# rst-tu-dortmund/teb_local_planner

Measured on NVIDIA B200. Metric: TEB trajectories/sec (complete optimizeTEB: outer x inner LM iterations + cost), higher is better.
Workload: dtype f64

## Files before the change

teb_local_planner_b200/csrc/teb_cabi.cu:

```cuda
#include <cuda_runtime.h>

#include <cmath>
#include <cstdio>
#include <cstring>
#include <new>
#include <string>
#include <vector>

#include "teb_kernels.cuh"
#include "teb_linearize.cuh"
#include "teb_spec.cuh"
#include "teb_solve_warp.cuh"
#include "teb_solve_lat.cuh"
#include "teb_hsig.cuh"
#include "teb_comm.h"
#include <cstdlib>

using namespace tebgpu;

struct tebgpu_ctx {
  int device = 0;
  cudaStream_t stream = nullptr;
  cudaStream_t side = nullptr;
  cudaEvent_t ev_fork = nullptr, ev_join = nullptr, ev_s0 = nullptr;
// ... 4 lines not shown
  int32_t* defer = nullptr;
  double* d_fp = nullptr;
  double* d_pverts = nullptr;
  double* d_hsig = nullptr;
  TebGpuLimits lim{};
  TebParams params{};
  bool have_params = false;
  std::string err;
  int64_t launches = 0;
  int linearize_variant = 0;
  ncclComm_t comm = nullptr;
  int world = 1, rank = 0;
  int32_t* arrive = nullptr;
  int eval_mode = 2;
  double* d_gather = nullptr;
  struct GraphEntry { uint64_t key = 0; cudaGraphExec_t exec = nullptr; int64_t launches = 0; uint64_t stamp = 0; int spec_k = 0, spec_first = 0; };
  std::vector<GraphEntry> graphs;
  uint64_t graph_clock = 0;
  uint64_t params_version = 0;
  int graph_mode = 2;
  int warp_solver = 4;
  int ring = 0;
  int eval_v1 = 0;
  int ka_staged = 1;
  int last_spec_k = 0;
  int last_spec_first = 0;
  int spec_k = 0;
  int solver = 2;
  int MW = 1;
  int chunks = 1;
  double* Hb = nullptr;
  unsigned long long* assoc = nullptr;
  unsigned long long* assoc3 = nullptr;
  double* dyn_t = nullptr;
  int32_t* via_idx = nullptr;
  double* chi_parts = nullptr;
  double* dmax_parts = nullptr;
  double* rhs = nullptr;
  int32_t* dyn_idx = nullptr;
  int32_t* dyn_cnt = nullptr;
  SpecBufs spec{};
  int eval_minb = 3;
  BandState* state = nullptr;
  double* d_poses = nullptr; int32_t* d_n = nullptr; int32_t* d_scene = nullptr; TebObstacle* d_obst = nullptr;
  int32_t* d_ocount = nullptr; double* d_via = nullptr; int32_t* d_vcount = nullptr; double* d_vs = nullptr;
  double* d_vg = nullptr; int32_t* d_rot = nullptr; double* d_cost = nullptr; double* d_chi2 = nullptr;
  int32_t* d_status = nullptr; int32_t* d_iters = nullptr;
// ... 203 lines not shown
  CUDA_TRY(c, cudaMalloc(&c->d_pverts, (S * (size_t)(lim->max_obst_vertices > 0 ? lim->max_obst_vertices : 1)) * 2 * sizeof(double)));
  CUDA_TRY(c, cudaMalloc(&c->d_hsig, B * (M > 2 ? M : 2) * sizeof(double)));
  CUDA_TRY(c, cudaMalloc(&c->d_vcount, B * sizeof(int32_t)));
  CUDA_TRY(c, cudaMalloc(&c->d_vs, B * 4 * sizeof(double)));
  CUDA_TRY(c, cudaMalloc(&c->d_vg, B * 4 * sizeof(double)));
  CUDA_TRY(c, cudaMalloc(&c->d_rot, B * sizeof(int32_t)));
  CUDA_TRY(c, cudaMalloc(&c->d_cost, B * sizeof(double)));
  CUDA_TRY(c, cudaMalloc(&c->d_chi2, B * sizeof(double)));
  CUDA_TRY(c, cudaMalloc(&c->d_status, B * sizeof(int32_t)));
  CUDA_TRY(c, cudaMalloc(&c->d_iters, B * sizeof(int32_t)));
  CUDA_TRY(c, cudaMemsetAsync(c->dyn_t, 0, B * nc * sizeof(double), c->stream));
  CUDA_TRY(c, cudaMemsetAsync(c->via_idx, 0xff, B * V * sizeof(int32_t), c->stream));
  c->smem_a = ka_smem_bytes((int)M);
  c->smem_b = kb_smem_bytes((int)nc, (int)M);
  c->smem_g = M * sizeof(TebObstacle);
  if (c->smem_b > 232448 || c->smem_a > 232448) {
    c->err = "shared-memory footprint exceeds 227 KB for these limits (max_poses / max_obstacles too large)";
    return TEBGPU_ERR_CAPACITY;
  }
  if (ka2_smem_bytes<true>((int)M) > 232448) {
    c->err = "kernel A staging exceeds 227 KB for these limits (max_obstacles too large)";
    return TEBGPU_ERR_CAPACITY;
  }
#define KA2_ATTR(H, G, O)                                                                                                    \
  CUDA_TRY(c, cudaFuncSetAttribute(k_linearize2<H, G, O>, cudaFuncAttributeMaxDynamicSharedMemorySize, (int)ka2_smem_bytes<H>((int)M))); \
  CUDA_TRY(c, cudaFuncSetAttribute(k_linearize2<H, G, O>, cudaFuncAttributePreferredSharedMemoryCarveout, cudaSharedmemCarveoutMaxShared));
  KA2_ATTR(false, false, true) KA2_ATTR(false, true, true) KA2_ATTR(true, false, true) KA2_ATTR(true, true, true)
  KA2_ATTR(false, false, false) KA2_ATTR(false, true, false) KA2_ATTR(true, false, false) KA2_ATTR(true, true, false)
#undef KA2_ATTR
  c->ka_staged = 1;
  if (const char* e = std::getenv("TEBGPU_KA_STAGED")) c->ka_staged = std::atoi(e) != 0;
  CUDA_TRY(c, cudaFuncSetAttribute(k_linearize<false, false>, cudaFuncAttributeMaxDynamicSharedMemorySize, (int)c->smem_a));
  CUDA_TRY(c, cudaFuncSetAttribute(k_linearize<false, true>, cudaFuncAttributeMaxDynamicSharedMemorySize, (int)c->smem_a));
  CUDA_TRY(c, cudaFuncSetAttribute(k_linearize<true, false>, cudaFuncAttributeMaxDynamicSharedMemorySize, (int)c->smem_a));
  CUDA_TRY(c, cudaFuncSetAttribute(k_linearize<true, true>, cudaFuncAttributeMaxDynamicSharedMemorySize, (int)c->smem_a));
  CUDA_TRY(c, cudaFuncSetAttribute(k_lm_step_t<0, KB_THREADS, false>, cudaFuncAttributeMaxDynamicSharedMemorySize, (int)c->smem_b));
  CUDA_TRY(c, cudaFuncSetAttribute(k_lm_step_t<0, KB_THREADS, true>, cudaFuncAttributeMaxDynamicSharedMemorySize, (int)c->smem_b));
  if ((int)nc <= BCR_MAX_POSES && kb_bcr_smem_bytes((int)nc, (int)M) <= 232448) {
    CUDA_TRY(c, cudaFuncSetAttribute(k_lm_step_t<1, KB_BCR_THREADS, false>, cudaFuncAttributeMaxDynamicSharedMemorySize,
                                     (int)kb_bcr_smem_bytes((int)nc, (int)M)));
    CUDA_TRY(c, cudaFuncSetAttribute(k_lm_step_t<1, KB_BCR_THREADS, true>, cudaFuncAttributeMaxDynamicSharedMemorySize,
                                     (int)kb_bcr_smem_bytes((int)nc, (int)M)));
  }
  CUDA_TRY(c, cudaFuncSetAttribute(k_build_graph<false>, cudaFuncAttributeMaxDynamicSharedMemorySize, (int)c->smem_g));
  CUDA_TRY(c, cudaFuncSetAttribute(k_build_graph<true>, cudaFuncAttributeMaxDynamicSharedMemorySize, (int)c->smem_g));
  CUDA_TRY(c, cudaFuncSetAttribute(k_linearize<false, false>, cudaFuncAttributePreferredSharedMemoryCarveout, cudaSharedmemCarveoutMaxShared));
  CUDA_TRY(c, cudaFuncSetAttribute(k_linearize<false, true>, cudaFuncAttributePreferredSharedMemoryCarveout, cudaSharedmemCarveoutMaxShared));
  CUDA_TRY(c, cudaFuncSetAttribute(k_linearize<true, false>, cudaFuncAttributePreferredSharedMemoryCarveout, cudaSharedmemCarveoutMaxShared));
  CUDA_TRY(c, cudaFuncSetAttribute(k_linearize<true, true>, cudaFuncAttributePreferredSharedMemoryCarveout, cudaSharedmemCarveoutMaxShared));
  CUDA_TRY(c, cudaFuncSetAttribute(k_solve_tpb<10>, cudaFuncAttributePreferredSharedMemoryCarveout, cudaSharedmemCarveoutMaxShared));
  CUDA_TRY(c, cudaFuncSetAttribute(k_solve_tpb<20>, cudaFuncAttributePreferredSharedMemoryCarveout, cudaSharedmemCarveoutMaxShared));
  CUDA_TRY(c, cudaFuncSetAttribute(k_solve_tpb<30>, cudaFuncAttributePreferredSharedMemoryCarveout, cudaSharedmemCarveoutMaxShared));
  CUDA_TRY(c, cudaFuncSetAttribute(k_solve_tpb<20>, cudaFuncAttributeMaxDynamicSharedMemorySize, tpb_ring_bytes(20)));
  CUDA_TRY(c, cudaFuncSetAttribute(k_solve_tpb<30>, cudaFuncAttributeMaxDynamicSharedMemorySize, tpb_ring_bytes(30)));
// ... 49 lines not shown
  for (int k = 0; k < 4; ++k) fp[FP_LINE + k] = p->footprint_line[k];
  fp[FP_COUNT] = (double)p->footprint_vertex_count;
  for (int k = 0; k < 2 * TEB_MAX_FOOTPRINT_VERTICES; ++k) fp[FP_VERTS + k] = p->footprint_vertices[k];
  CUDA_TRY(ctx, cudaSetDevice(ctx->device));
  CUDA_TRY(ctx, cudaStreamSynchronize(ctx->stream));
  CUDA_TRY(ctx, cudaMemcpy(ctx->d_fp, fp, sizeof(fp), cudaMemcpyHostToDevice));
  ctx->params = *p;
  ctx->have_params = true;
  ++ctx->params_version;
  return TEBGPU_OK;
}

static void launch_linearize(tebgpu_ctx* ctx, const DevBatch& db, const KParams& kp, int B, int M_cap, cudaStream_t st) {
  const bool holo = kp.holo_vel || kp.holo_acc;
  const bool geom = kp.generic != 0;
  if (ctx->linearize_variant == 1) {
    const dim3 grid(db.chunks, B);
    const size_t sm = ka_smem_bytes(M_cap);
    if (holo && geom) k_linearize<true, true><<<grid, KA_THREADS, sm, st>>>(db, kp);
    else if (holo) k_linearize<true, false><<<grid, KA_THREADS, sm, st>>>(db, kp);
    else if (geom) k_linearize<false, true><<<grid, KA_THREADS, sm, st>>>(db, kp);
    else k_linearize<false, false><<<grid, KA_THREADS, sm, st>>>(db, kp);
  } else {
    const dim3 g2((db.chunks + KA2_W - 1) / KA2_W, B);
    const size_t sm = holo ? ka2_smem_bytes<true>(M_cap) : ka2_smem_bytes<false>(M_cap);
#define KA2_LAUNCH(H, G)                                                                      \
  do {                                                                                        \
    if (ctx->ka_staged) k_linearize2<H, G, false><<<g2, KA2_THREADS, sm, st>>>(db, kp);       \
    else k_linearize2<H, G, true><<<g2, KA2_THREADS, sm, st>>>(db, kp);                       \
  } while (0)
    if (holo && geom) KA2_LAUNCH(true, true);
    else if (holo) KA2_LAUNCH(true, false);
    else if (geom) KA2_LAUNCH(false, true);
    else KA2_LAUNCH(false, false);
#undef KA2_LAUNCH
  }
}
static void launch_build_graph(const DevBatch& db, const KParams& kp, int B, size_t smem, cudaStream_t st) {
  if (kp.generic) k_build_graph<true><<<B, 256, smem, st>>>(db, kp);
  else k_build_graph<false><<<B, 256, smem, st>>>(db, kp);
}
static void launch_vor(const DevBatch& db, const KParams& kp, int B, size_t smem, cudaStream_t st) {
  if (kp.generic) k_vor<true><<<B, 256, smem, st>>>(db, kp);
  else k_vor<false><<<B, 256, smem, st>>>(db, kp);
}
static size_t eval_bytes(const tebgpu_ctx* ctx, int n_cap, int M_cap, int K) {
  return ctx->eval_v1 ? eval_smem_bytes(n_cap, M_cap, K) : eval2_smem_bytes(n_cap, M_cap, K);
}
static void launch_trial_eval(tebgpu_ctx* ctx, const SpecBufs& spec, const DevBatch& db, const KParams& kp, int B, int K,
                              size_t smem, int it, int round, int g, int tag, cudaStream_t st) {
  const size_t smem3 = eval3_smem_bytes(db.n_cap, db.M_cap, K);
  if (!ctx->eval_v1 && smem3 <= 232448 && (ctx->eval_mode == 1 || (ctx->eval_mode == 2 && (long long)B * K <= 148 * 3))) {
    int warps = ev2_tiles(db.n_cap);
    warps = warps < 1 ? 1 : (warps > 16 ? 16 : warps);
    const dim3 grid(K, B);
    if (kp.generic) k_trial_eval3<true><<<grid, 32 * warps, smem3, st>>>(db, kp, spec, it, round, g, tag, ctx->arrive);
    else k_trial_eval3<false><<<grid, 32 * warps, smem3, st>>>(db, kp, spec, it, round, g, tag, ctx->arrive);
    return;
// ... 262 lines not shown
        else if (kp.generic) k_lm_step_t<0, KB_THREADS, true><<<B, KB_THREADS, smem_b, st>>>(db, kp, it);
        else k_lm_step_t<0, KB_THREADS, false><<<B, KB_THREADS, smem_b, st>>>(db, kp, it);
        ++launches; prof_end(ctx, st);
      }
    }
    weight_multiplier *= p.weight_adapt_factor;
  }
  prof_begin(ctx, st, 5); k_finalize<<<gb, tb, 0, st>>>(db, kp, *args); ++launches; prof_end(ctx, st);
  ctx->launches = launches;
  if (ctx->profiling && ctx->ev_used > 4096) { cudaStreamSynchronize(st); prof_collect(ctx); }
  CUDA_TRY(ctx, cudaGetLastError());
  return TEBGPU_OK;
}

static uint64_t graph_key(const tebgpu_ctx* ctx, const TebBatch* bt, const TebOptimizeArgs* a, cudaStream_t st) {
  uint64_t h = 1469598103934665603ull;
  auto mix = [&](const void* p, size_t nbytes) {
    const unsigned char* c = static_cast<const unsigned char*>(p);
    for (size_t k = 0; k < nbytes; ++k) { h ^= c[k]; h *= 1099511628211ull; }
  };
  mix(bt, sizeof(*bt));
  mix(a, sizeof(*a));
  mix(&ctx->params_version, sizeof(ctx->params_version));
  const int sw[11] = {ctx->solver, ctx->spec_k, ctx->linearize_variant, ctx->ka_staged, ctx->eval_v1, ctx->ring, ctx->overlap, ctx->eval_minb, ctx->warp_solver, ctx->eval_mode, ctx->split};
  mix(sw, sizeof(sw));
  mix(&st, sizeof(st));
  return h;
}

int32_t tebgpu_optimize_batch_device(tebgpu_ctx* ctx, const TebBatch* bt, const TebOptimizeArgs* args, void* cuda_stream) {
  int32_t rc = check_batch(ctx, bt);
  if (rc) return rc;
  if (!args || args->iterations_innerloop < 0 || args->iterations_outerloop < 0) { ctx->err = "bad optimize args"; return TEBGPU_ERR_INVALID_ARG; }
  CUDA_TRY(ctx, cudaSetDevice(ctx->device));
  cudaStream_t st = cuda_stream ? (cudaStream_t)cuda_stream : ctx->stream;
  const bool latency_regime = (long long)bt->B * 8 <= 148LL * 4 * 32;
  const bool use_graph = !ctx->profiling && (ctx->graph_mode == 1 || (ctx->graph_mode == 2 && latency_regime));
  if (!use_graph) return issue_optimize(ctx, bt, args, st);
  const uint64_t key = graph_key(ctx, bt, args, st);
  for (auto& e : ctx->graphs)
    if (e.key == key) {
      e.stamp = ++ctx->graph_clock;
      ctx->launches = e.launches;
      ctx->last_spec_k = e.spec_k; ctx->last_spec_first = e.spec_first;
      CUDA_TRY(ctx, cudaGraphLaunch(e.exec, st));
      return TEBGPU_OK;
    }
// ... 431 lines not shown
```

teb_local_planner_b200/csrc/teb_linearize.cuh:

```cuda
#pragma once

#include "teb_kernels.cuh"

namespace tebgpu {

constexpr int KA2_W = 4;
constexpr int KA2_THREADS = 32 * KA2_W;
constexpr int KA2_TP = 29;
constexpr int KA2_SLOTS = KA2_W * KA2_TP + 4;
constexpr int KA2_NT = 32;
constexpr int OUT_STRIDE = 50;

template <bool HOLO>
struct JL {
  static constexpr int V = 0;
  static constexpr int W = V + 7;
  static constexpr int K0 = W + 3;
  static constexpr int K1 = K0 + 6;
  static constexpr int SP = K1 + 6;
  static constexpr int ROT = SP + 4;
  static constexpr int VY = ROT + 2;
  static constexpr int A0 = VY + (HOLO ? 6 : 0);
  static constexpr int A1 = A0 + 11;
  static constexpr int A2 = A1 + 5;
  static constexpr int E = A2 + (HOLO ? 11 : 0);
  static constexpr int COUNT = E + (HOLO ? 10 : 8);
};
constexpr unsigned M_V = 0x7Fu, M_W = (1u << 2) | (1u << 3) | (1u << 6), M_K = 0x77u, M_SP = 0x33u,
                   M_ROT = (1u << 2) | (1u << 6), M_VY = 0x3Fu, M_A0 = 0x7FFu,
                   M_A1 = (1u << 2) | (1u << 3) | (1u << 6) | (1u << 7) | (1u << 10);
enum { E_V = 0, E_W = 1, E_K0 = 2, E_K1 = 3, E_SP = 4, E_ROT = 5, E_A0 = 6, E_A1 = 7, E_VY = 8, E_A2 = 9 };

__host__ __device__ constexpr int cidx(unsigned mask, int col) {
  int k = 0;
  for (int c = 0; c < col; ++c) k += (mask >> c) & 1u;
  return k;
}

struct JRec {
  double* rec;
  template <int BASE, unsigned MASK, int COL>
  __device__ __forceinline__ void set(double v) const {
    if constexpr ((MASK >> COL) & 1u) rec[(BASE + cidx(MASK, COL)) * KA2_NT] = v;
  }
  __device__ __forceinline__ void res(int base_e, int k, double v) const { rec[(base_e + k) * KA2_NT] = v; }
};

struct KA2Smem {
  static constexpr int POSES = KA2_SLOTS * 4;
  static constexpr int START = 24;
  template <bool HOLO>
  __host__ __device__ static constexpr int rec_doubles() {
    return JL<HOLO>::COUNT * 32 > OUT_STRIDE * 32 ? JL<HOLO>::COUNT * 32 : OUT_STRIDE * 32;
  }
  template <bool HOLO>
  __host__ __device__ static constexpr int warp_doubles() { return rec_doubles<HOLO>() + START; }
};
template <bool HOLO>
__host__ __device__ inline size_t ka2_smem_bytes(int M_cap) {
  const size_t d = KA2Smem::POSES + (size_t)KA2_W * KA2Smem::warp_doubles<HOLO>() + 2;
  return d * sizeof(double) + (size_t)(M_cap > 0 ? M_cap : 1) * sizeof(TebObstacle) + 64;
}

template <bool HOLO>
__device__ __forceinline__ double anchor_rows2(const KParams& kp, const DevBatch& db, int b, int a, int n,
                                               const double* pa , double ca, double sa, double cb,
                                               double sb, const SegDer& sd, const SegDer& sd2, const JRec J,
                                               double* sStart) {
  using L = JL<HOLO>;
  const double* pb = pa + 4;
  const double v1 = sd.v, w1 = sd.w, idt1 = sd.idt;
  const double dx = pb[0] - pa[0], dy = pb[1] - pa[1];
  const bool fa = (a == 0), fb = (a + 1 == n - 1);
  const double ma = fa ? 0.0 : 1.0, mb = fb ? 0.0 : 1.0;
  double csum = 0;
  if (HOLO && kp.has_vel && kp.holo_vel) {
    const HoloDer h = holo_derivs(pa[0], pa[1], pa[2], ca, sa, pb[0], pb[1], pb[2], pa[3]);
    double e[3], sl[3], c0, c1;
    holo_velocity_terms(kp, h.vx, h.vy, h.w, e, sl, c0, c1);
    const double kx = kp.sw_vel_x, ky = kp.sw_vel_y, kw = kp.sw_vel_th * sl[2];
    J.set<L::V, M_V, 0>(ma * kx * (sl[0] * h.dvx[0] - c0 * h.dvy[0]));
    J.set<L::V, M_V, 1>(ma * kx * (sl[0] * h.dvx[1] - c0 * h.dvy[1]));
    J.set<L::V, M_V, 2>(ma * kx * (sl[0] * h.dvx[2] - c0 * h.dvy[2]));
// ... 225 lines not shown
      if (vs[3] != 0) {
        const double acc = (v1 - vs[0]) * idt1;
        const double accr = (w1 - vs[2]) * idt1;
        double s0, s1;
        const double e0 = pen_interval(acc, kp.p.acc_lim_x, kp.p.penalty_epsilon, s0);
        const double e1 = pen_interval(accr, kp.p.acc_lim_theta, kp.p.penalty_epsilon, s1);
        const double k0 = kp.sw_acc_x * s0 * idt1, k1 = kp.sw_acc_th * s1 * idt1;
        double* S0 = sStart;
        double* S1 = sStart + 7;
        S0[0] = 0; S0[1] = 0; S0[2] = 0;
        S0[3] = k0 * (-v1 * idt1 - acc);
        S0[4] = k0 * sd.dv[3] * mb; S0[5] = k0 * sd.dv[4] * mb; S0[6] = k0 * sd.dv[5] * mb;
        S1[0] = S1[1] = S1[2] = S1[4] = S1[5] = 0;
        S1[3] = k1 * (-w1 * idt1 - accr);
        S1[6] = k1 * idt1 * mb;
        sStart[START_E] = kp.sw_acc_x * e0; sStart[START_E + 1] = kp.sw_acc_th * e1;
        csum += sStart[START_E] * sStart[START_E] + sStart[START_E + 1] * sStart[START_E + 1];
      }
    }
  }
  return csum;
}

template <int D, int BASE, unsigned MASK, int NC>
__device__ __forceinline__ void gram_row(const double* __restrict__ jr_base, double e, double (&acc)[4][11], double (&brow)[4]) {
  constexpr int LMAX = (4 * D + 3 < NC - 1) ? 4 * D + 3 : NC - 1;
  if constexpr (4 * D < NC) {
    double jr[NC];
#pragma unroll
    for (int col = 0; col < NC; ++col) jr[col] = (((MASK >> col) & 1u) && col <= LMAX) ? jr_base[(BASE + cidx(MASK, col)) * KA2_NT] : 0.0;
#pragma unroll
    for (int c = 0; c < 4; ++c) {
      const int l = 4 * D + c;
      if (l < NC && ((MASK >> l) & 1u)) {
        const double jl = jr[l];
        brow[c] -= jl * e;
#pragma unroll
        for (int o = 0; o <= 10; ++o) {
          const int col = l - o;
          if (col >= 0 && ((MASK >> col) & 1u)) acc[c][o] += jl * jr[col];
        }
      }
    }
  }
}

template <bool HOLO, int D>
__device__ __forceinline__ void gram_anchor(const KParams& kp, const double* __restrict__ jr_base, double (&acc)[4][11],
                                            double (&brow)[4]) {
  using L = JL<HOLO>;
  const double* E = jr_base + L::E * KA2_NT;
  if (D < 2) {
    if (kp.has_vel) {
      const double ev = E[E_V * KA2_NT], ew = E[E_W * KA2_NT];
      if (ev != 0) gram_row<D, L::V, M_V, 7>(jr_base, ev, acc, brow);
      if (ew != 0) gram_row<D, L::W, M_W, 7>(jr_base, ew, acc, brow);
      if (HOLO) {
        const double ey = E[E_VY * KA2_NT];
        if (ey != 0) gram_row<D, L::VY, M_VY, 6>(jr_base, ey, acc, brow);
      }
    }
    if (kp.has_kin) {
      const double e0 = E[E_K0 * KA2_NT], e1 = E[E_K1 * KA2_NT];
      if (e0 != 0) gram_row<D, L::K0, M_K, 7>(jr_base, e0, acc, brow);
      if (e1 != 0) gram_row<D, L::K1, M_K, 7>(jr_base, e1, acc, brow);
    }
    if (kp.has_sp) {
      const double e = E[E_SP * KA2_NT];
      if (e != 0) gram_row<D, L::SP, M_SP, 6>(jr_base, e, acc, brow);
    }
    if (kp.has_rot) {
      const double e = E[E_ROT * KA2_NT];
      if (e != 0) gram_row<D, L::ROT, M_ROT, 7>(jr_base, e, acc, brow);
    }
  }
  if (kp.has_acc) {
    const double e0 = E[E_A0 * KA2_NT], e1 = E[E_A1 * KA2_NT];
    if (e0 != 0) gram_row<D, L::A0, M_A0, 11>(jr_base, e0, acc, brow);
    if (e1 != 0) gram_row<D, L::A1, M_A1, 11>(jr_base, e1, acc, brow);
    if (HOLO) {
      const double e2 = E[E_A2 * KA2_NT];
      if (e2 != 0) gram_row<D, L::A2, M_A0, 11>(jr_base, e2, acc, brow);
    }
  }
}

template <bool HOLO, int D>
__device__ __forceinline__ void gram_start(const double* sStart, double (&acc)[4][11], double (&brow)[4]) {
#pragma unroll
  for (int k = 0; k < (HOLO ? 3 : 2); ++k) {
    const double e = sStart[START_E + k];
    if (e == 0) continue;
#pragma unroll
    for (int c = 0; c < 4; ++c) {
      const int l = 4 * D + c;
      if (l <= 6) {
        const double jl = sStart[7 * k + l];
        brow[c] -= jl * e;
#pragma unroll
        for (int o = 0; o <= 6; ++o)
          if (o <= l) acc[c][o] += jl * sStart[7 * k + l - o];
      }
    }
  }
}

template <bool GEOM>
__device__ __forceinline__ void unary_terms2(const KParams& kp, const DevBatch& db, int b, int sc, int i, int n, double px,
                                             double py, double cs, double sn, const TebObstacle* so, unsigned long long mask0,
                                             double U[6], double ub[3], double& chi_obst, double& chi_via) {
  if (i < 1 || i > n - 2) return;
  const double* pool = db.obst_vertices + (size_t)sc * db.PV_cap * 2;
  if (kp.has_obst) {
    const unsigned long long* assoc = db.assoc + ((size_t)b * db.n_cap + i) * db.MW;
    for (int w = 0; w < db.MW; ++w) {
      unsigned long long mask = (w == 0) ? mask0 : assoc[w];
      while (mask) {
        const int m = (w << 6) + __ffsll((long long)mask) - 1;
        mask &= mask - 1;
        const TebObstacle ob = so[m];
        double g[3], kappa, beta;
        const double d = robot_obstacle_distance<GEOM>(kp, pool, px, py, cs, sn, ob, ob.x, ob.y, 0.0, 0.0, g);
        double cterm = obstacle_terms(kp, d, kappa, beta);
        if (kp.p.legacy_obstacle_association &&
            ((db.assoc3[((size_t)b * db.n_cap + i) * db.MW + w] >> (m & 63)) & 1ull)) {
          cterm *= 3; kappa *= 3; beta *= 3;
        }
        chi_obst += cterm;
        if (kappa != 0 || beta != 0) {
          U[0] += kappa * g[0] * g[0]; U[1] += kappa * g[0] * g[1]; U[2] += kappa * g[1] * g[1];
          U[3] += kappa * g[0] * g[2]; U[4] += kappa * g[1] * g[2]; U[5] += kappa * g[2] * g[2];
          ub[0] -= beta * g[0]; ub[1] -= beta * g[1]; ub[2] -= beta * g[2];
        }
      }
    }
  }
  if (kp.has_dyn) {
    const double t = db.dyn_t[(size_t)b * db.n_cap + i];
    const int nd = db.dyn_cnt[sc];
    const int32_t* di = db.dyn_idx + (size_t)sc * db.M_cap;
    for (int q = 0; q < nd; ++q) {
      const TebObstacle ob = so[di[q]];
      double g[3], kappa, beta;
      const double d = robot_obstacle_distance<GEOM>(kp, pool, px, py, cs, sn, ob, ob.x + t * ob.vx, ob.y + t * ob.vy, t * ob.vx,
                                               t * ob.vy, g);
      chi_obst += dynamic_terms(kp, d, kappa, beta);
      if (kappa != 0 || beta != 0) {
        U[0] += kappa * g[0] * g[0]; U[1] += kappa * g[0] * g[1]; U[2] += kappa * g[1] * g[1];
        U[3] += kappa * g[0] * g[2]; U[4] += kappa * g[1] * g[2]; U[5] += kappa * g[2] * g[2];
        ub[0] -= beta * g[0]; ub[1] -= beta * g[1]; ub[2] -= beta * g[2];
      }
    }
  }
  if (kp.has_via && db.V_cap > 0) {
    const int32_t* vidx = db.via_idx + (size_t)b * db.V_cap;
    const double* via = db.via + (size_t)b * db.V_cap * 2;
    const double wv = kp.p.weight_viapoint;
    for (int v = 0; v < db.V_cap; ++v) {
      if (vidx[v] != i) continue;
      const double dx = px - via[2 * v], dy = py - via[2 * v + 1];
      const double e = sqrt(dx * dx + dy * dy);
      chi_via += wv * e * e;
      if (e > 0) {
        const double gx = dx / e, gy = dy / e;
        U[0] += wv * gx * gx; U[1] += wv * gx * gy; U[2] += wv * gy * gy;
        ub[0] -= wv * e * gx; ub[1] -= wv * e * gy;
      }
    }
  }
}

__device__ __forceinline__ double shfl_down1(double v) { return __shfl_down_sync(0xffffffffu, v, 1); }

template <bool HOLO, bool GEOM, bool OUT_DIRECT>
__global__ void __launch_bounds__(KA2_THREADS, 3) k_linearize2(const __grid_constant__ DevBatch db, const __grid_constant__ KParams kp) {
  extern __shared__ __align__(128) unsigned char smem_raw[];
  using L = JL<HOLO>;
  const int tid = threadIdx.x, lane = tid & 31, warp = tid >> 5;
  double* sP = reinterpret_cast<double*>(smem_raw);
  double* sW = sP + KA2Smem::POSES + (size_t)warp * KA2Smem::warp_doubles<HOLO>();
  double* sStart = sW + KA2Smem::rec_doubles<HOLO>();
  uint64_t* bar = reinterpret_cast<uint64_t*>(sP + KA2Smem::POSES + (size_t)KA2_W * KA2Smem::warp_doubles<HOLO>());
  TebObstacle* so = reinterpret_cast<TebObstacle*>((reinterpret_cast<uintptr_t>(bar) + 16 + 15) & ~static_cast<uintptr_t>(15));

  const int y = blockIdx.y;
  int b = y, skip = 0;
  if (db.a_list) { if (y < *db.a_cnt) b = db.a_list[y]; else skip = 1; }
  else if (db.skip_tag != 0 && deferred_since(db.defer[y], db.skip_tag)) skip = 1;
  if (skip) return;
  const int active = db.state[b].active;
  const int n = db.n[b];
  const int s = db.scene_id[b];
  const int P0 = blockIdx.x * (KA2_W * KA2_TP) - 2;
  const int lo = max(P0, 0), hi = min(P0 + KA2_SLOTS, db.n_cap);
  if (tid == 0) {
    mbar_init(bar, 1);
    mbar_fence_init();
  }
  if (!active || P0 + 2 >= n) return;
  if (tid == 0) {
    const uint32_t bytesP = (uint32_t)(hi - lo) * 32u;
    const uint32_t bytesO = (uint32_t)db.M_cap * (uint32_t)sizeof(TebObstacle);
    mbar_expect_tx(bar, bytesP + bytesO);
    tma_load_1d(sP + (size_t)(lo - P0) * 4, db.poses + ((size_t)b * db.n_cap + lo) * 4, bytesP, bar);
    if (bytesO) tma_load_1d(so, db.obstacles + (size_t)s * db.M_cap, bytesO, bar);
  }
  const int slot = warp * KA2_TP + lane;
  const int i = P0 + slot;
  const int q0 = P0 + 2 + warp * KA2_TP;
  const bool out = (lane >= 2 && lane <= 30 && i < n);
  unsigned long long mask0 = 0ull;
  if (out && kp.has_obst && i >= 1 && i <= n - 2) mask0 = db.assoc[((size_t)b * db.n_cap + i) * db.MW];
  {
    double* rec = sW + lane;
#pragma unroll
    for (int e = 0; e < L::COUNT; ++e) rec[e * 32] = 0.0;
    if (lane < KA2Smem::START) sStart[lane] = 0.0;
  }
  __syncthreads();
  mbar_wait(bar, 0);
  if (q0 >= n) return;

  double chi[4] = {0, 0, 0, 0};
  const bool have_pose = (i >= 0 && i < n);
  const double* pa = sP + 4 * slot;
  double cs = 1, sn = 0;
  SegDer sd;
  sd.v = 0; sd.w = 0; sd.idt = 0;
#pragma unroll
  for (int k = 0; k < 6; ++k) sd.dv[k] = 0;
  double U[6] = {0, 0, 0, 0, 0, 0}, ub[3] = {0, 0, 0};
  if (have_pose) {
    sincos(pa[2], &sn, &cs);
    if (i <= n - 2) sd = seg_derivs(kp, pa[0], pa[1], pa[2], cs, sn, pa[4], pa[5], pa[6], pa[3]);
    if (out) unary_terms2<GEOM>(kp, db, b, s, i, n, pa[0], pa[1], cs, sn, so, mask0, U, ub, chi[0], chi[1]);
  }
  SegDer sd2;
  const double cb = shfl_down1(cs), sb = shfl_down1(sn);
  sd2.v = shfl_down1(sd.v); sd2.w = shfl_down1(sd.w); sd2.idt = shfl_down1(sd.idt);
#pragma unroll
  for (int k = 0; k < 6; ++k) sd2.dv[k] = shfl_down1(sd.dv[k]);
  __syncwarp();
  if (have_pose && i <= n - 2 && lane < 31) {
    JRec J;
    J.rec = sW + lane;
    const double c3 = anchor_rows2<HOLO>(kp, db, b, i, n, pa, cs, sn, cb, sb, sd, sd2, J, sStart);
    if (lane >= 2) chi[3] += c3;
  }
  __syncwarp();
  double acc[4][11];
  double brow[4] = {0, 0, 0, 0};
#pragma unroll
  for (int c = 0; c < 4; ++c)
#pragma unroll
    for (int k = 0; k < 11; ++k) acc[c][k] = 0;
  double dm = 0;
  if (out) {
    const double* rec = sW + lane;
    if (i <= n - 2) gram_anchor<HOLO, 0>(kp, rec, acc, brow);
    if (i >= 1) gram_anchor<HOLO, 1>(kp, rec - 1, acc, brow);
    if (i >= 2) gram_anchor<HOLO, 2>(kp, rec - 2, acc, brow);
    if (kp.has_acc) {
      if (i == 0) gram_start<HOLO, 0>(sStart, acc, brow);
      if (i == 1) gram_start<HOLO, 1>(sStart, acc, brow);
    }
    acc[0][0] += U[0]; brow[0] += ub[0];
    acc[1][0] += U[2]; acc[1][1] += U[1]; brow[1] += ub[1];
    acc[2][0] += U[5]; acc[2][1] += U[4]; acc[2][2] += U[3]; brow[2] += ub[2];
    if (kp.has_time && i <= n - 2) {
      chi[2] += kp.p.weight_optimaltime * pa[3] * pa[3];
      acc[3][0] += kp.p.weight_optimaltime; brow[3] -= kp.p.weight_optimaltime * pa[3];
    }
    if (i == 0 || i >= n - 1) {
#pragma unroll
      for (int c = 0; c < 4; ++c) {
        if (c == 3 && i <= n - 2) continue;
#pragma unroll
        for (int k = 0; k < 11; ++k) acc[c][k] = 0;
        acc[c][0] = 1.0;
        brow[c] = 0;
      }
      dm = (i <= n - 2) ? fabs(acc[3][0]) : 0.0;
    } else {
      dm = fmax(fmax(fabs(acc[0][0]), fabs(acc[1][0])), fmax(fabs(acc[2][0]), fabs(acc[3][0])));
    }
  }
  if (OUT_DIRECT) {
    if (out) {
      double2* g2 = reinterpret_cast<double2*>(db.Hb + ((size_t)b * 4 * db.n_cap + 4 * (size_t)i) * HROW);
#pragma unroll
      for (int c = 0; c < 4; ++c) {
#pragma unroll
        for (int k = 0; k < 5; ++k) g2[6 * c + k] = make_double2(acc[c][2 * k], acc[c][2 * k + 1]);
        g2[6 * c + 5] = make_double2(acc[c][10], brow[c]);
      }
      double2* r2 = reinterpret_cast<double2*>(db.rhs + (size_t)b * 4 * db.n_cap + 4 * (size_t)i);
      r2[0] = make_double2(brow[0], brow[1]);
      r2[1] = make_double2(brow[2], brow[3]);
    }
  } else {
    __syncwarp();
    if (out) {
      double2* o2 = reinterpret_cast<double2*>(sW + (size_t)lane * OUT_STRIDE);
#pragma unroll
      for (int c = 0; c < 4; ++c) {
#pragma unroll
        for (int k = 0; k < 5; ++k) o2[6 * c + k] = make_double2(acc[c][2 * k], acc[c][2 * k + 1]);
        o2[6 * c + 5] = make_double2(acc[c][10], brow[c]);
      }
      double2* r2 = reinterpret_cast<double2*>(db.rhs + (size_t)b * 4 * db.n_cap + 4 * (size_t)i);
      r2[0] = make_double2(brow[0], brow[1]);
      r2[1] = make_double2(brow[2], brow[3]);
      fence_proxy_async();
      tma_store_1d(db.Hb + ((size_t)b * 4 * db.n_cap + 4 * (size_t)i) * HROW, o2, 4 * HROW * 8u);
      asm volatile("cp.async.bulk.commit_group;" ::: "memory");
    }
  }
  {
#pragma unroll
    for (int k = 0; k < 4; ++k) chi[k] = warp_sum(chi[k]);
    dm = warp_max(dm);
    if (lane == 0) {
      const int tile = blockIdx.x * KA2_W + warp;
      double* cp = db.chi_parts + ((size_t)b * db.chunks + tile) * 4;
      cp[0] = chi[0]; cp[1] = chi[1]; cp[2] = chi[2]; cp[3] = chi[3];
      db.dmax_parts[(size_t)b * db.chunks + tile] = dm;
    }
  }
  if (!OUT_DIRECT && out) asm volatile("cp.async.bulk.wait_group.read 0;" ::: "memory");
}

}
```

Before: 171,100.

## Split linearize tile work across warp pairs with role-specialized warps

Restructures the linearization kernel so each 29-pose tile is handled by a pair of warps instead of one. One warp computes the segment derivatives and anchor Jacobian rows, while the other computes the obstacle unary terms. Each warp then builds two of the four Gram rows and writes them with its own bulk store. Named barriers and a shared exchange buffer pass the unary block and the diagonal max between the two warps. The change also evaluates obstacles two at a time for more instruction-level parallelism, raises the min-CTA launch bounds, and drops the direct-output variant and its environment switch. It aims to cut per-thread register pressure and serial latency, at the cost of more shared memory, extra barriers and more CTAs.

```diff
diff --git a/teb_local_planner_b200/csrc/teb_cabi.cu b/teb_local_planner_b200/csrc/teb_cabi.cu
--- a/teb_local_planner_b200/csrc/teb_cabi.cu
+++ b/teb_local_planner_b200/csrc/teb_cabi.cu
@@ -50,7 +50,6 @@
   int warp_solver = 4;
   int ring = 0;
   int eval_v1 = 0;
-  int ka_staged = 1;
   int last_spec_k = 0;
   int last_spec_first = 0;
   int spec_k = 0;
@@ -300,14 +299,11 @@
     c->err = "kernel A staging exceeds 227 KB for these limits (max_obstacles too large)";
     return TEBGPU_ERR_CAPACITY;
   }
-#define KA2_ATTR(H, G, O)                                                                                                    \
-  CUDA_TRY(c, cudaFuncSetAttribute(k_linearize2<H, G, O>, cudaFuncAttributeMaxDynamicSharedMemorySize, (int)ka2_smem_bytes<H>((int)M))); \
-  CUDA_TRY(c, cudaFuncSetAttribute(k_linearize2<H, G, O>, cudaFuncAttributePreferredSharedMemoryCarveout, cudaSharedmemCarveoutMaxShared));
-  KA2_ATTR(false, false, true) KA2_ATTR(false, true, true) KA2_ATTR(true, false, true) KA2_ATTR(true, true, true)
-  KA2_ATTR(false, false, false) KA2_ATTR(false, true, false) KA2_ATTR(true, false, false) KA2_ATTR(true, true, false)
+#define KA2_ATTR(H, G)                                                                                                    \
+  CUDA_TRY(c, cudaFuncSetAttribute(k_linearize2<H, G>, cudaFuncAttributeMaxDynamicSharedMemorySize, (int)ka2_smem_bytes<H>((int)M))); \
+  CUDA_TRY(c, cudaFuncSetAttribute(k_linearize2<H, G>, cudaFuncAttributePreferredSharedMemoryCarveout, cudaSharedmemCarveoutMaxShared));
+  KA2_ATTR(false, false) KA2_ATTR(false, true) KA2_ATTR(true, false) KA2_ATTR(true, true)
 #undef KA2_ATTR
-  c->ka_staged = 1;
-  if (const char* e = std::getenv("TEBGPU_KA_STAGED")) c->ka_staged = std::atoi(e) != 0;
   CUDA_TRY(c, cudaFuncSetAttribute(k_linearize<false, false>, cudaFuncAttributeMaxDynamicSharedMemorySize, (int)c->smem_a));
   CUDA_TRY(c, cudaFuncSetAttribute(k_linearize<false, true>, cudaFuncAttributeMaxDynamicSharedMemorySize, (int)c->smem_a));
   CUDA_TRY(c, cudaFuncSetAttribute(k_linearize<true, false>, cudaFuncAttributeMaxDynamicSharedMemorySize, (int)c->smem_a));
@@ -403,18 +399,12 @@
     else if (geom) k_linearize<false, true><<<grid, KA_THREADS, sm, st>>>(db, kp);
     else k_linearize<false, false><<<grid, KA_THREADS, sm, st>>>(db, kp);
   } else {
-    const dim3 g2((db.chunks + KA2_W - 1) / KA2_W, B);
+    const dim3 g2((db.chunks + KA2_P - 1) / KA2_P, B);
     const size_t sm = holo ? ka2_smem_bytes<true>(M_cap) : ka2_smem_bytes<false>(M_cap);
-#define KA2_LAUNCH(H, G)                                                                      \
-  do {                                                                                        \
-    if (ctx->ka_staged) k_linearize2<H, G, false><<<g2, KA2_THREADS, sm, st>>>(db, kp);       \
-    else k_linearize2<H, G, true><<<g2, KA2_THREADS, sm, st>>>(db, kp);                       \
-  } while (0)
-    if (holo && geom) KA2_LAUNCH(true, true);
-    else if (holo) KA2_LAUNCH(true, false);
-    else if (geom) KA2_LAUNCH(false, true);
-    else KA2_LAUNCH(false, false);
-#undef KA2_LAUNCH
+    if (holo && geom) k_linearize2<true, true><<<g2, KA2_THREADS, sm, st>>>(db, kp);
+    else if (holo) k_linearize2<true, false><<<g2, KA2_THREADS, sm, st>>>(db, kp);
+    else if (geom) k_linearize2<false, true><<<g2, KA2_THREADS, sm, st>>>(db, kp);
+    else k_linearize2<false, false><<<g2, KA2_THREADS, sm, st>>>(db, kp);
   }
 }
 static void launch_build_graph(const DevBatch& db, const KParams& kp, int B, size_t smem, cudaStream_t st) {
@@ -723,7 +713,7 @@
   mix(bt, sizeof(*bt));
   mix(a, sizeof(*a));
   mix(&ctx->params_version, sizeof(ctx->params_version));
-  const int sw[11] = {ctx->solver, ctx->spec_k, ctx->linearize_variant, ctx->ka_staged, ctx->eval_v1, ctx->ring, ctx->overlap, ctx->eval_minb, ctx->warp_solver, ctx->eval_mode, ctx->split};
+  const int sw[10] = {ctx->solver, ctx->spec_k, ctx->linearize_variant, ctx->eval_v1, ctx->ring, ctx->overlap, ctx->eval_minb, ctx->warp_solver, ctx->eval_mode, ctx->split};
   mix(sw, sizeof(sw));
   mix(&st, sizeof(st));
   return h;
diff --git a/teb_local_planner_b200/csrc/teb_linearize.cuh b/teb_local_planner_b200/csrc/teb_linearize.cuh
--- a/teb_local_planner_b200/csrc/teb_linearize.cuh
+++ b/teb_local_planner_b200/csrc/teb_linearize.cuh
@@ -4,10 +4,12 @@
 
 namespace tebgpu {
 
-constexpr int KA2_W = 4;
-constexpr int KA2_THREADS = 32 * KA2_W;
+constexpr int KA2_P = 2;
+constexpr int KA2_THREADS = 64 * KA2_P;
+template <bool GEOM>
+constexpr int ka2_min_ctas() { return GEOM ? 4 : 5; }
 constexpr int KA2_TP = 29;
-constexpr int KA2_SLOTS = KA2_W * KA2_TP + 4;
+constexpr int KA2_SLOTS = KA2_P * KA2_TP + 4;
 constexpr int KA2_NT = 32;
 constexpr int OUT_STRIDE = 50;
 
@@ -49,16 +51,19 @@
 struct KA2Smem {
   static constexpr int POSES = KA2_SLOTS * 4;
   static constexpr int START = 24;
+  static constexpr int XCH = 6 * 32;
   template <bool HOLO>
   __host__ __device__ static constexpr int rec_doubles() {
     return JL<HOLO>::COUNT * 32 > OUT_STRIDE * 32 ? JL<HOLO>::COUNT * 32 : OUT_STRIDE * 32;
   }
   template <bool HOLO>
-  __host__ __device__ static constexpr int warp_doubles() { return rec_doubles<HOLO>() + START; }
+  __host__ __device__ static constexpr int pair_doubles() { return rec_doubles<HOLO>() + START + XCH; }
 };
+static_assert(KA2Smem::POSES % 2 == 0 && KA2Smem::pair_doubles<false>() % 2 == 0 && KA2Smem::pair_doubles<true>() % 2 == 0,
+              "output slots must stay 16-byte aligned for the bulk stores");
 template <bool HOLO>
 __host__ __device__ inline size_t ka2_smem_bytes(int M_cap) {
-  const size_t d = KA2Smem::POSES + (size_t)KA2_W * KA2Smem::warp_doubles<HOLO>() + 2;
+  const size_t d = KA2Smem::POSES + (size_t)KA2_P * KA2Smem::pair_doubles<HOLO>() + 2;
   return d * sizeof(double) + (size_t)(M_cap > 0 ? M_cap : 1) * sizeof(TebObstacle) + 64;
 }
 
@@ -330,86 +335,106 @@
   return csum;
 }
 
-template <int D, int BASE, unsigned MASK, int NC>
-__device__ __forceinline__ void gram_row(const double* __restrict__ jr_base, double e, double (&acc)[4][11], double (&brow)[4]) {
-  constexpr int LMAX = (4 * D + 3 < NC - 1) ? 4 * D + 3 : NC - 1;
-  if constexpr (4 * D < NC) {
+template <int D, int R0, int BASE, unsigned MASK, int NC>
+__device__ __forceinline__ void gram_row(const double* __restrict__ jr_base, double e, double (&acc)[2][11], double (&brow)[2]) {
+  constexpr int LMAX = (4 * D + R0 + 1 < NC - 1) ? 4 * D + R0 + 1 : NC - 1;
+  if constexpr (4 * D + R0 < NC) {
     double jr[NC];
 #pragma unroll
     for (int col = 0; col < NC; ++col) jr[col] = (((MASK >> col) & 1u) && col <= LMAX) ? jr_base[(BASE + cidx(MASK, col)) * KA2_NT] : 0.0;
 #pragma unroll
-    for (int c = 0; c < 4; ++c) {
-      const int l = 4 * D + c;
+    for (int cc = 0; cc < 2; ++cc) {
+      const int l = 4 * D + R0 + cc;
       if (l < NC && ((MASK >> l) & 1u)) {
         const double jl = jr[l];
-        brow[c] -= jl * e;
+        brow[cc] -= jl * e;
 #pragma unroll
         for (int o = 0; o <= 10; ++o) {
           const int col = l - o;
-          if (col >= 0 && ((MASK >> col) & 1u)) acc[c][o] += jl * jr[col];
+          if (col >= 0 && ((MASK >> col) & 1u)) acc[cc][o] += jl * jr[col];
         }
       }
     }
   }
 }
 
-template <bool HOLO, int D>
-__device__ __forceinline__ void gram_anchor(const KParams& kp, const double* __restrict__ jr_base, double (&acc)[4][11],
-                                            double (&brow)[4]) {
+template <bool HOLO, int D, int R0>
+__device__ __forceinline__ void gram_anchor(const KParams& kp, const double* __restrict__ jr_base, double (&acc)[2][11],
+                                            double (&brow)[2]) {
   using L = JL<HOLO>;
   const double* E = jr_base + L::E * KA2_NT;
   if (D < 2) {
     if (kp.has_vel) {
       const double ev = E[E_V * KA2_NT], ew = E[E_W * KA2_NT];
-      if (ev != 0) gram_row<D, L::V, M_V, 7>(jr_base, ev, acc, brow);
-      if (ew != 0) gram_row<D, L::W, M_W, 7>(jr_base, ew, acc, brow);
+      if (ev != 0) gram_row<D, R0, L::V, M_V, 7>(jr_base, ev, acc, brow);
+      if (ew != 0) gram_row<D, R0, L::W, M_W, 7>(jr_base, ew, acc, brow);
       if (HOLO) {
         const double ey = E[E_VY * KA2_NT];
-        if (ey != 0) gram_row<D, L::VY, M_VY, 6>(jr_base, ey, acc, brow);
+        if (ey != 0) gram_row<D, R0, L::VY, M_VY, 6>(jr_base, ey, acc, brow);
       }
     }
     if (kp.has_kin) {
       const double e0 = E[E_K0 * KA2_NT], e1 = E[E_K1 * KA2_NT];
-      if (e0 != 0) gram_row<D, L::K0, M_K, 7>(jr_base, e0, acc, brow);
-      if (e1 != 0) gram_row<D, L::K1, M_K, 7>(jr_base, e1, acc, brow);
+      if (e0 != 0) gram_row<D, R0, L::K0, M_K, 7>(jr_base, e0, acc, brow);
+      if (e1 != 0) gram_row<D, R0, L::K1, M_K, 7>(jr_base, e1, acc, brow);
     }
     if (kp.has_sp) {
       const double e = E[E_SP * KA2_NT];
-      if (e != 0) gram_row<D, L::SP, M_SP, 6>(jr_base, e, acc, brow);
+      if (e != 0) gram_row<D, R0, L::SP, M_SP, 6>(jr_base, e, acc, brow);
     }
     if (kp.has_rot) {
       const double e = E[E_ROT * KA2_NT];
-      if (e != 0) gram_row<D, L::ROT, M_ROT, 7>(jr_base, e, acc, brow);
+      if (e != 0) gram_row<D, R0, L::ROT, M_ROT, 7>(jr_base, e, acc, brow);
     }
   }
   if (kp.has_acc) {
     const double e0 = E[E_A0 * KA2_NT], e1 = E[E_A1 * KA2_NT];
-    if (e0 != 0) gram_row<D, L::A0, M_A0, 11>(jr_base, e0, acc, brow);
-    if (e1 != 0) gram_row<D, L::A1, M_A1, 11>(jr_base, e1, acc, brow);
+    if (e0 != 0) gram_row<D, R0, L::A0, M_A0, 11>(jr_base, e0, acc, brow);
+    if (e1 != 0) gram_row<D, R0, L::A1, M_A1, 11>(jr_base, e1, acc, brow);
     if (HOLO) {
       const double e2 = E[E_A2 * KA2_NT];
-      if (e2 != 0) gram_row<D, L::A2, M_A0, 11>(jr_base, e2, acc, brow);
-    }
-  }
-}
-
-template <bool HOLO, int D>
-__device__ __forceinline__ void gram_start(const double* sStart, double (&acc)[4][11], double (&brow)[4]) {
+      if (e2 != 0) gram_row<D, R0, L::A2, M_A0, 11>(jr_base, e2, acc, brow);
+    }
+  }
+}
+
+template <bool HOLO, int D, int R0>
+__device__ __forceinline__ void gram_start(const double* sStart, double (&acc)[2][11], double (&brow)[2]) {
 #pragma unroll
   for (int k = 0; k < (HOLO ? 3 : 2); ++k) {
     const double e = sStart[START_E + k];
     if (e == 0) continue;
 #pragma unroll
-    for (int c = 0; c < 4; ++c) {
-      const int l = 4 * D + c;
+    for (int cc = 0; cc < 2; ++cc) {
+      const int l = 4 * D + R0 + cc;
       if (l <= 6) {
         const double jl = sStart[7 * k + l];
-        brow[c] -= jl * e;
+        brow[cc] -= jl * e;
 #pragma unroll
         for (int o = 0; o <= 6; ++o)
-          if (o <= l) acc[c][o] += jl * sStart[7 * k + l - o];
-      }
-    }
+          if (o <= l) acc[cc][o] += jl * sStart[7 * k + l - o];
+      }
+    }
+  }
+}
+
+template <bool HOLO, int R0>
+__device__ __forceinline__ void gram_rows(const KParams& kp, const double* rec, const double* sStart, int i, int n,
+                                          double (&acc)[2][11], double (&brow)[2]) {
+  if (i <= n - 2) gram_anchor<HOLO, 0, R0>(kp, rec, acc, brow);
+  if (i >= 1) gram_anchor<HOLO, 1, R0>(kp, rec - 1, acc, brow);
+  if (i >= 2) gram_anchor<HOLO, 2, R0>(kp, rec - 2, acc, brow);
+  if (kp.has_acc) {
+    if (i == 0) gram_start<HOLO, 0, R0>(sStart, acc, brow);
+    if (i == 1) gram_start<HOLO, 1, R0>(sStart, acc, brow);
+  }
+}
+
+__device__ __forceinline__ void add_unary_block(double kappa, double beta, const double g[3], double U[6], double ub[3]) {
+  if (kappa != 0 || beta != 0) {
+    U[0] += kappa * g[0] * g[0]; U[1] += kappa * g[0] * g[1]; U[2] += kappa * g[1] * g[1];
+    U[3] += kappa * g[0] * g[2]; U[4] += kappa * g[1] * g[2]; U[5] += kappa * g[2] * g[2];
+    ub[0] -= beta * g[0]; ub[1] -= beta * g[1]; ub[2] -= beta * g[2];
   }
 }
 
@@ -423,22 +448,26 @@
     const unsigned long long* assoc = db.assoc + ((size_t)b * db.n_cap + i) * db.MW;
     for (int w = 0; w < db.MW; ++w) {
       unsigned long long mask = (w == 0) ? mask0 : assoc[w];
+      const unsigned long long l3 = kp.p.legacy_obstacle_association ? db.assoc3[((size_t)b * db.n_cap + i) * db.MW + w] : 0ull;
       while (mask) {
-        const int m = (w << 6) + __ffsll((long long)mask) - 1;
+        const int m1 = (w << 6) + __ffsll((long long)mask) - 1;
         mask &= mask - 1;
-        const TebObstacle ob = so[m];
-        double g[3], kappa, beta;
-        const double d = robot_obstacle_distance<GEOM>(kp, pool, px, py, cs, sn, ob, ob.x, ob.y, 0.0, 0.0, g);
-        double cterm = obstacle_terms(kp, d, kappa, beta);
-        if (kp.p.legacy_obstacle_association &&
-            ((db.assoc3[((size_t)b * db.n_cap + i) * db.MW + w] >> (m & 63)) & 1ull)) {
-          cterm *= 3; kappa *= 3; beta *= 3;
-        }
-        chi_obst += cterm;
-        if (kappa != 0 || beta != 0) {
-          U[0] += kappa * g[0] * g[0]; U[1] += kappa * g[0] * g[1]; U[2] += kappa * g[1] * g[1];
-          U[3] += kappa * g[0] * g[2]; U[4] += kappa * g[1] * g[2]; U[5] += kappa * g[2] * g[2];
-          ub[0] -= beta * g[0]; ub[1] -= beta * g[1]; ub[2] -= beta * g[2];
+        const bool two = mask != 0;
+        const int m2 = two ? (w << 6) + __ffsll((long long)mask) - 1 : m1;
+        if (two) mask &= mask - 1;
+        const TebObstacle o1 = so[m1], o2 = so[m2];
+        double g1[3], g2[3], k1, b1, k2, b2;
+        const double d1 = robot_obstacle_distance<GEOM>(kp, pool, px, py, cs, sn, o1, o1.x, o1.y, 0.0, 0.0, g1);
+        const double d2 = robot_obstacle_distance<GEOM>(kp, pool, px, py, cs, sn, o2, o2.x, o2.y, 0.0, 0.0, g2);
+        double c1 = obstacle_terms(kp, d1, k1, b1);
+        double c2 = obstacle_terms(kp, d2, k2, b2);
+        if ((l3 >> (m1 & 63)) & 1ull) { c1 *= 3; k1 *= 3; b1 *= 3; }
+        if ((l3 >> (m2 & 63)) & 1ull) { c2 *= 3; k2 *= 3; b2 *= 3; }
+        chi_obst += c1;
+        add_unary_block(k1, b1, g1, U, ub);
+        if (two) {
+          chi_obst += c2;
+          add_unary_block(k2, b2, g2, U, ub);
         }
       }
     }
@@ -453,11 +482,7 @@
       const double d = robot_obstacle_distance<GEOM>(kp, pool, px, py, cs, sn, ob, ob.x + t * ob.vx, ob.y + t * ob.vy, t * ob.vx,
                                                t * ob.vy, g);
       chi_obst += dynamic_terms(kp, d, kappa, beta);
-      if (kappa != 0 || beta != 0) {
-        U[0] += kappa * g[0] * g[0]; U[1] += kappa * g[0] * g[1]; U[2] += kappa * g[1] * g[1];
-        U[3] += kappa * g[0] * g[2]; U[4] += kappa * g[1] * g[2]; U[5] += kappa * g[2] * g[2];
-        ub[0] -= beta * g[0]; ub[1] -= beta * g[1]; ub[2] -= beta * g[2];
-      }
+      add_unary_block(kappa, beta, g, U, ub);
     }
   }
   if (kp.has_via && db.V_cap > 0) {
@@ -480,15 +505,23 @@
 
 __device__ __forceinline__ double shfl_down1(double v) { return __shfl_down_sync(0xffffffffu, v, 1); }
 
-template <bool HOLO, bool GEOM, bool OUT_DIRECT>
-__global__ void __launch_bounds__(KA2_THREADS, 3) k_linearize2(const __grid_constant__ DevBatch db, const __grid_constant__ KParams kp) {
+static_assert(KA2_P == 2, "pair_sync names one barrier per pair");
+__device__ __forceinline__ void pair_sync(int p) {
+  if (p == 0) asm volatile("bar.sync 1, 64;" ::: "memory");
+  else asm volatile("bar.sync 2, 64;" ::: "memory");
+}
+
+template <bool HOLO, bool GEOM>
+__global__ void __launch_bounds__(KA2_THREADS, ka2_min_ctas<GEOM>()) k_linearize2(const __grid_constant__ DevBatch db, const __grid_constant__ KParams kp) {
   extern __shared__ __align__(128) unsigned char smem_raw[];
   using L = JL<HOLO>;
   const int tid = threadIdx.x, lane = tid & 31, warp = tid >> 5;
+  const int pair = warp >> 1, role = warp & 1;
   double* sP = reinterpret_cast<double*>(smem_raw);
-  double* sW = sP + KA2Smem::POSES + (size_t)warp * KA2Smem::warp_doubles<HOLO>();
+  double* sW = sP + KA2Smem::POSES + (size_t)pair * KA2Smem::pair_doubles<HOLO>();
   double* sStart = sW + KA2Smem::rec_doubles<HOLO>();
-  uint64_t* bar = reinterpret_cast<uint64_t*>(sP + KA2Smem::POSES + (size_t)KA2_W * KA2Smem::warp_doubles<HOLO>());
+  double* sX = sStart + KA2Smem::START;
+  uint64_t* bar = reinterpret_cast<uint64_t*>(sP + KA2Smem::POSES + (size_t)KA2_P * KA2Smem::pair_doubles<HOLO>());
   TebObstacle* so = reinterpret_cast<TebObstacle*>((reinterpret_cast<uintptr_t>(bar) + 16 + 15) & ~static_cast<uintptr_t>(15));
 
   const int y = blockIdx.y;
@@ -499,7 +532,7 @@
   const int active = db.state[b].active;
   const int n = db.n[b];
   const int s = db.scene_id[b];
-  const int P0 = blockIdx.x * (KA2_W * KA2_TP) - 2;
+  const int P0 = blockIdx.x * (KA2_P * KA2_TP) - 2;
   const int lo = max(P0, 0), hi = min(P0 + KA2_SLOTS, db.n_cap);
   if (tid == 0) {
     mbar_init(bar, 1);
@@ -513,17 +546,19 @@
     tma_load_1d(sP + (size_t)(lo - P0) * 4, db.poses + ((size_t)b * db.n_cap + lo) * 4, bytesP, bar);
     if (bytesO) tma_load_1d(so, db.obstacles + (size_t)s * db.M_cap, bytesO, bar);
   }
-  const int slot = warp * KA2_TP + lane;
+  const int slot = pair * KA2_TP + lane;
   const int i = P0 + slot;
-  const int q0 = P0 + 2 + warp * KA2_TP;
+  const int q0 = P0 + 2 + pair * KA2_TP;
   const bool out = (lane >= 2 && lane <= 30 && i < n);
   unsigned long long mask0 = 0ull;
-  if (out && kp.has_obst && i >= 1 && i <= n - 2) mask0 = db.assoc[((size_t)b * db.n_cap + i) * db.MW];
+  if (role == 1 && out && kp.has_obst && i >= 1 && i <= n - 2) mask0 = db.assoc[((size_t)b * db.n_cap + i) * db.MW];
   {
+    constexpr int HALF = (L::COUNT + 1) / 2;
     double* rec = sW + lane;
 #pragma unroll
-    for (int e = 0; e < L::COUNT; ++e) rec[e * 32] = 0.0;
-    if (lane < KA2Smem::START) sStart[lane] = 0.0;
+    for (int e = 0; e < HALF; ++e)
+      if (role * HALF + e < L::COUNT) rec[(role * HALF + e) * 32] = 0.0;
+    if (role == 0 && lane < KA2Smem::START) sStart[lane] = 0.0;
   }
   __syncthreads();
   mbar_wait(bar, 0);
@@ -532,110 +567,113 @@
   double chi[4] = {0, 0, 0, 0};
   const bool have_pose = (i >= 0 && i < n);
   const double* pa = sP + 4 * slot;
-  double cs = 1, sn = 0;
-  SegDer sd;
-  sd.v = 0; sd.w = 0; sd.idt = 0;
-#pragma unroll
-  for (int k = 0; k < 6; ++k) sd.dv[k] = 0;
   double U[6] = {0, 0, 0, 0, 0, 0}, ub[3] = {0, 0, 0};
-  if (have_pose) {
-    sincos(pa[2], &sn, &cs);
-    if (i <= n - 2) sd = seg_derivs(kp, pa[0], pa[1], pa[2], cs, sn, pa[4], pa[5], pa[6], pa[3]);
-    if (out) unary_terms2<GEOM>(kp, db, b, s, i, n, pa[0], pa[1], cs, sn, so, mask0, U, ub, chi[0], chi[1]);
-  }
-  SegDer sd2;
-  const double cb = shfl_down1(cs), sb = shfl_down1(sn);
-  sd2.v = shfl_down1(sd.v); sd2.w = shfl_down1(sd.w); sd2.idt = shfl_down1(sd.idt);
-#pragma unroll
-  for (int k = 0; k < 6; ++k) sd2.dv[k] = shfl_down1(sd.dv[k]);
-  __syncwarp();
-  if (have_pose && i <= n - 2 && lane < 31) {
-    JRec J;
-    J.rec = sW + lane;
-    const double c3 = anchor_rows2<HOLO>(kp, db, b, i, n, pa, cs, sn, cb, sb, sd, sd2, J, sStart);
-    if (lane >= 2) chi[3] += c3;
-  }
-  __syncwarp();
-  double acc[4][11];
-  double brow[4] = {0, 0, 0, 0};
-#pragma unroll
-  for (int c = 0; c < 4; ++c)
+  if (role == 0) {
+    double cs = 1, sn = 0;
+    SegDer sd;
+    sd.v = 0; sd.w = 0; sd.idt = 0;
+#pragma unroll
+    for (int k = 0; k < 6; ++k) sd.dv[k] = 0;
+    if (have_pose) {
+      sincos(pa[2], &sn, &cs);
+      if (i <= n - 2) sd = seg_derivs(kp, pa[0], pa[1], pa[2], cs, sn, pa[4], pa[5], pa[6], pa[3]);
+    }
+    SegDer sd2;
+    const double cb = shfl_down1(cs), sb = shfl_down1(sn);
+    sd2.v = shfl_down1(sd.v); sd2.w = shfl_down1(sd.w); sd2.idt = shfl_down1(sd.idt);
+#pragma unroll
+    for (int k = 0; k < 6; ++k) sd2.dv[k] = shfl_down1(sd.dv[k]);
+    if (have_pose && i <= n - 2 && lane < 31) {
+      JRec J;
+      J.rec = sW + lane;
+      const double c3 = anchor_rows2<HOLO>(kp, db, b, i, n, pa, cs, sn, cb, sb, sd, sd2, J, sStart);
+      if (lane >= 2) chi[3] += c3;
+    }
+  } else {
+    if (out && i >= 1 && i <= n - 2) {
+      double cs, sn;
+      sincos(pa[2], &sn, &cs);
+      unary_terms2<GEOM>(kp, db, b, s, i, n, pa[0], pa[1], cs, sn, so, mask0, U, ub, chi[0], chi[1]);
+    }
+    sX[0 * 32 + lane] = U[0]; sX[1 * 32 + lane] = U[1]; sX[2 * 32 + lane] = U[2];
+    sX[3 * 32 + lane] = ub[0]; sX[4 * 32 + lane] = ub[1];
+  }
+  pair_sync(pair);
+  double acc[2][11];
+  double brow[2] = {0, 0};
+#pragma unroll
+  for (int c = 0; c < 2; ++c)
 #pragma unroll
     for (int k = 0; k < 11; ++k) acc[c][k] = 0;
   double dm = 0;
+  const bool fixed_rows = (i == 0 || i >= n - 1);
   if (out) {
     const double* rec = sW + lane;
-    if (i <= n - 2) gram_anchor<HOLO, 0>(kp, rec, acc, brow);
-    if (i >= 1) gram_anchor<HOLO, 1>(kp, rec - 1, acc, brow);
-    if (i >= 2) gram_anchor<HOLO, 2>(kp, rec - 2, acc, brow);
-    if (kp.has_acc) {
-      if (i == 0) gram_start<HOLO, 0>(sStart, acc, brow);
-      if (i == 1) gram_start<HOLO, 1>(sStart, acc, brow);
-    }
-    acc[0][0] += U[0]; brow[0] += ub[0];
-    acc[1][0] += U[2]; acc[1][1] += U[1]; brow[1] += ub[1];
-    acc[2][0] += U[5]; acc[2][1] += U[4]; acc[2][2] += U[3]; brow[2] += ub[2];
-    if (kp.has_time && i <= n - 2) {
-      chi[2] += kp.p.weight_optimaltime * pa[3] * pa[3];
-      acc[3][0] += kp.p.weight_optimaltime; brow[3] -= kp.p.weight_optimaltime * pa[3];
-    }
-    if (i == 0 || i >= n - 1) {
-#pragma unroll
-      for (int c = 0; c < 4; ++c) {
-        if (c == 3 && i <= n - 2) continue;
-#pragma unroll
-        for (int k = 0; k < 11; ++k) acc[c][k] = 0;
-        acc[c][0] = 1.0;
-        brow[c] = 0;
-      }
-      dm = (i <= n - 2) ? fabs(acc[3][0]) : 0.0;
+    if (role == 0) {
+      gram_rows<HOLO, 0>(kp, rec, sStart, i, n, acc, brow);
+      acc[0][0] += sX[0 * 32 + lane]; brow[0] += sX[3 * 32 + lane];
+      acc[1][0] += sX[2 * 32 + lane]; acc[1][1] += sX[1 * 32 + lane]; brow[1] += sX[4 * 32 + lane];
+      if (fixed_rows) {
+#pragma unroll
+        for (int c = 0; c < 2; ++c) {
+#pragma unroll
+          for (int k = 0; k < 11; ++k) acc[c][k] = 0;
+          acc[c][0] = 1.0;
+          brow[c] = 0;
+        }
+      }
     } else {
-      dm = fmax(fmax(fabs(acc[0][0]), fabs(acc[1][0])), fmax(fabs(acc[2][0]), fabs(acc[3][0])));
-    }
-  }
-  if (OUT_DIRECT) {
-    if (out) {
-      double2* g2 = reinterpret_cast<double2*>(db.Hb + ((size_t)b * 4 * db.n_cap + 4 * (size_t)i) * HROW);
-#pragma unroll
-      for (int c = 0; c < 4; ++c) {
-#pragma unroll
-        for (int k = 0; k < 5; ++k) g2[6 * c + k] = make_double2(acc[c][2 * k], acc[c][2 * k + 1]);
-        g2[6 * c + 5] = make_double2(acc[c][10], brow[c]);
-      }
-      double2* r2 = reinterpret_cast<double2*>(db.rhs + (size_t)b * 4 * db.n_cap + 4 * (size_t)i);
-      r2[0] = make_double2(brow[0], brow[1]);
-      r2[1] = make_double2(brow[2], brow[3]);
-    }
+      gram_rows<HOLO, 2>(kp, rec, sStart, i, n, acc, brow);
+      acc[0][0] += U[5]; acc[0][1] += U[4]; acc[0][2] += U[3]; brow[0] += ub[2];
+      if (kp.has_time && i <= n - 2) {
+        chi[2] += kp.p.weight_optimaltime * pa[3] * pa[3];
+        acc[1][0] += kp.p.weight_optimaltime; brow[1] -= kp.p.weight_optimaltime * pa[3];
+      }
+      if (fixed_rows) {
+#pragma unroll
+        for (int c = 0; c < 2; ++c) {
+          if (c == 1 && i <= n - 2) continue;
+#pragma unroll
+          for (int k = 0; k < 11; ++k) acc[c][k] = 0;
+          acc[c][0] = 1.0;
+          brow[c] = 0;
+        }
+        dm = (i <= n - 2) ? fabs(acc[1][0]) : 0.0;
+      }
+    }
+    if (role == 0 && !fixed_rows) sX[5 * 32 + lane] = fmax(fabs(acc[0][0]), fabs(acc[1][0]));
+  }
+  pair_sync(pair);
+  if (out) {
+    if (role == 1 && !fixed_rows) dm = fmax(sX[5 * 32 + lane], fmax(fabs(acc[0][0]), fabs(acc[1][0])));
+    double2* o2 = reinterpret_cast<double2*>(sW + (size_t)lane * OUT_STRIDE + 2 * HROW * role);
+#pragma unroll
+    for (int c = 0; c < 2; ++c) {
+#pragma unroll
+      for (int k = 0; k < 5; ++k) o2[6 * c + k] = make_double2(acc[c][2 * k], acc[c][2 * k + 1]);
+      o2[6 * c + 5] = make_double2(acc[c][10], brow[c]);
+    }
+    double2* r2 = reinterpret_cast<double2*>(db.rhs + (size_t)b * 4 * db.n_cap + 4 * (size_t)i + 2 * role);
+    r2[0] = make_double2(brow[0], brow[1]);
+    fence_proxy_async();
+    tma_store_1d(db.Hb + ((size_t)b * 4 * db.n_cap + 4 * (size_t)i + 2 * role) * HROW, o2, 2 * HROW * 8u);
+    asm volatile("cp.async.bulk.commit_group;" ::: "memory");
+  }
+  const int tile = blockIdx.x * KA2_P + pair;
+  double* cp = db.chi_parts + ((size_t)b * db.chunks + tile) * 4;
+  if (role == 0) {
+    chi[3] = warp_sum(chi[3]);
+    if (lane == 0) cp[3] = chi[3];
   } else {
-    __syncwarp();
-    if (out) {
-      double2* o2 = reinterpret_cast<double2*>(sW + (size_t)lane * OUT_STRIDE);
-#pragma unroll
-      for (int c = 0; c < 4; ++c) {
-#pragma unroll
-        for (int k = 0; k < 5; ++k) o2[6 * c + k] = make_double2(acc[c][2 * k], acc[c][2 * k + 1]);
-        o2[6 * c + 5] = make_double2(acc[c][10], brow[c]);
-      }
-      double2* r2 = reinterpret_cast<double2*>(db.rhs + (size_t)b * 4 * db.n_cap + 4 * (size_t)i);
-      r2[0] = make_double2(brow[0], brow[1]);
-      r2[1] = make_double2(brow[2], brow[3]);
-      fence_proxy_async();
-      tma_store_1d(db.Hb + ((size_t)b * 4 * db.n_cap + 4 * (size_t)i) * HROW, o2, 4 * HROW * 8u);
-      asm volatile("cp.async.bulk.commit_group;" ::: "memory");
-    }
-  }
-  {
-#pragma unroll
-    for (int k = 0; k < 4; ++k) chi[k] = warp_sum(chi[k]);
+#pragma unroll
+    for (int k = 0; k < 3; ++k) chi[k] = warp_sum(chi[k]);
     dm = warp_max(dm);
     if (lane == 0) {
-      const int tile = blockIdx.x * KA2_W + warp;
-      double* cp = db.chi_parts + ((size_t)b * db.chunks + tile) * 4;
-      cp[0] = chi[0]; cp[1] = chi[1]; cp[2] = chi[2]; cp[3] = chi[3];
+      cp[0] = chi[0]; cp[1] = chi[1]; cp[2] = chi[2];
       db.dmax_parts[(size_t)b * db.chunks + tile] = dm;
     }
   }
-  if (!OUT_DIRECT && out) asm volatile("cp.async.bulk.wait_group.read 0;" ::: "memory");
-}
-
-}
+  if (out) asm volatile("cp.async.bulk.wait_group.read 0;" ::: "memory");
+}
+
+}
```

Measured after the change: 166,300, median of 6. 0.972x the previous value.
